# dps/rust-raytracer

Measured on NVIDIA H100. Metric: Mrays/sec (primary+scattered), higher is better.
Workload: dtype f64

## Files before the change

rust-raytracer_b200/csrc/rtb200_api.cu:

```cuda
#include <algorithm>
#include <chrono>
#include <cmath>
#include <cstdio>
#include <cstdlib>
#include <cstring>
#include <mutex>
#include <string>
#include <thread>
#include <vector>

#include "rtb200_bvh.hpp"
#include "rtb200_kernels.cuh"

using namespace rtk;

static_assert(kCapIn >= 32 + 7 * rtbvh::kMaxDepth + 8, "the node stack must hold 32 roots plus a single-entry descent of the deepest tree (LIFO reserve, DESIGN.md 4.1)");

namespace {

thread_local std::string g_last_error;

int fail(int code, const std::string& msg) { g_last_error = msg; return code; }
int fail_cuda(cudaError_t e, const char* what) {
    g_last_error = std::string(what) + ": " + cudaGetErrorName(e) + " (" + cudaGetErrorString(e) + ")";
// ... 406 lines not shown
        const rt_image& im = s->textures[t];
        texs[t].rgb8 = nullptr; texs[t].width = im.width; texs[t].height = im.height;
        if (im.rgb8 && im.width && im.height && im.width * im.height * 3ull <= im.bytes)
            upload_array(h, im.rgb8, im.width * im.height * 3, (void**)&texs[t].rgb8);
    }
    upload_array(h, texs.data(), texs.size() * sizeof(rtd::DevTex), (void**)&tp.tex);
    tp.sky_mode = s->sky.mode;
    tp.sky.rgb8 = nullptr; tp.sky.width = 0; tp.sky.height = 0;
    if (s->sky.mode == RT_SKY_TEXTURE) {
        upload_array(h, s->sky.tex.rgb8, s->sky.tex.width * s->sky.tex.height * 3, (void**)&tp.sky.rgb8);
        tp.sky.width = s->sky.tex.width; tp.sky.height = s->sky.tex.height;
    }
    if (h->mode == MODE_TREE) { h->level_nodes = R.level_nodes; h->level_off = R.level_off; }
    std::vector<uint32_t> lights;
    for (uint32_t i = 0; i < n; ++i) {
        if (s->spheres[i].kind == RT_LIGHT) lights.push_back(i);
        if (albedo_nonfinite(s->spheres[i])) tp.albedo_nonfinite = 1u;
    }
    h->light_idx = lights;
    for (uint64_t t = 0; t < s->n_textures; ++t) h->tex_ok.push_back(image_ok(s->textures[t]));
    lights.push_back(0);
    upload_array(h, lights.data(), lights.size() * 4, (void**)&tp.lights);
    upload_array(h, nullptr, 16, (void**)&h->err);
    upload_array(h, nullptr, kMaxPending * kStatBytes, (void**)&h->stat_snap);
    tp.err = nullptr;
    tp.gx = R.g[0]; tp.gy = R.g[1]; tp.gz = R.g[2];
    tp.er_coef = 1.0f - (float)(96.0 * rtbvh::kU);
    tp.cam = s->camera;
    tp.width = s->width; tp.height = s->height; tp.spp = s->samples_per_pixel; tp.max_depth = s->max_depth;
    tp.key0 = (uint32_t)s->seed; tp.key1 = (uint32_t)(s->seed >> 32);
    tp.rank = opts.rank; tp.world = opts.world; tp.band_rows = opts.band_rows;
    tp.rows_local = rtb200_shard_rows(s->height, opts.rank, opts.world, opts.band_rows);
    tp.npix_local = tp.rows_local * s->width;

    const char* es = getenv("RTB200_WF_SMEM");
    tp.scene_in_smem = es ? (uint32_t)atoi(es) : 0u;
    h->smem = wavefront_smem_bytes(tp, h->mode, tp.scene_in_smem, Q_SINGLE);
    const int occ = occupancy(ctx, h->mode, n_lights > 0, Q_SINGLE, h->smem);
    if (occ <= 0) return fail(RT_ERR_UNSUPPORTED, "no launch configuration fits shared memory");
    h->ctas_per_sm = occ;
    h->grid = ctx->sm_count * occ;

    uint64_t cap = sample_buffer_cap(opts);
    uint64_t per_spp = (uint64_t)std::max<uint32_t>(tp.npix_local, 1) * 16ull;
    uint64_t spb = std::max<uint64_t>(1, cap / per_spp);
    spb = std::min<uint64_t>(spb, s->samples_per_pixel);
    while (spb > 1 && spb * tp.npix_local >= (1ull << 31)) spb /= 2;
    h->spp_batch = (uint32_t)spb;

    if ((rc = commit_uploads(h)) != RT_OK) return rc;
    h->tp.err = h->err;
    guard.ok = true;
    *out = h;
    return RT_OK;
}

int rtb200_scene_upload(const rt_scene* s, const rt_options* opts_in, rtb200_scene_handle* out) {
  return guarded([&]() -> int {
    if (!s || !out) return fail(RT_ERR_INVALID, "null argument");
    *out = nullptr;
    rt_options opts;
    int rc = normalise_options(opts_in, &opts);
    if (rc != RT_OK) return rc;
    uint32_t n_lights = 0;
    if ((rc = validate_scene(s, &n_lights)) != RT_OK) return rc;
    DeviceRestore restore;
// ... 976 lines not shown
```

rust-raytracer_b200/csrc/rtb200_kernels.cuh:

```cuda
#pragma once
#include <cuda_runtime.h>
#include <stdint.h>

#include "../../include/rtb200.h"
#include "rtb200_bvh.hpp"
#include "rtb200_device.cuh"

namespace rtk {

using rtbvh::kLeafK;
constexpr int kNodeVec = rtbvh::kNodeFloats / 4;
constexpr int kChildVec = rtbvh::kChildOff / 4;
using DevMat = rtbvh::Mat32;

#ifndef RT_BLOCK
#define RT_BLOCK 256
#endif
constexpr int kBlock = RT_BLOCK;
#ifndef RT_PHASE_CLOCKS
#define RT_PHASE_CLOCKS 0
#endif
enum : uint32_t { PH_HIT, PH_SORT_WAIT_A, PH_SHADE, PH_REGEN, PH_WAIT_C, PH_ITERS, PH_SCATTERS, PH_DEFERRED,
                  PH_NODE, PH_LEAF, PH_EXACT, PH_EXACT_STEPS, PH_EXACT_TESTS, PH_SRC_SKIPS, kPhaseN };
constexpr uint32_t kPhaseStat = 13;
#ifndef RT_CAP_IN
#define RT_CAP_IN 192
#endif
#ifndef RT_CAP_LF
#define RT_CAP_LF 160
#endif
#ifndef RT_CAP_CD
#define RT_CAP_CD 96
#endif
constexpr int kCapIn = RT_CAP_IN;
constexpr int kCapLf = RT_CAP_LF;
constexpr int kCapCd = RT_CAP_CD;

struct ShadowFrame {
    double px, py, pz;
    double ndx, ndy, ndz;
    float ar, ag, ab;
    float sr, sg, sb;
    uint32_t li, code, is_light, pad;
};
static_assert(sizeof(ShadowFrame) == 88, "ShadowFrame layout");

enum TraceMode : uint32_t { MODE_TREE = 0, MODE_BRUTE = 1, MODE_EXACT = 2 };
enum TraceQueue : uint32_t { Q_SINGLE = 0, Q_FRAMES = 1, Q_LIST = 2 };

struct FrameRec { rt_camera cam; uint32_t key0, key1; };
static_assert(sizeof(FrameRec) == 104, "FrameRec layout");

struct TraceParams {
    const float4*   nodes;
    const float4*   leaf_rec;
    const uint32_t* leaf_id;
    const uint32_t* skip_pos;
    const uint32_t* always;
    const float4*   filt;
    const double4*  geo;
    const DevMat*   mat;
    const rtd::DevTex* tex;
    uint32_t n, n_pairs, n_nodes, n_leaves, n_always, depth;
    uint32_t n_lights;
    uint32_t scene_in_smem;
    double gx, gy, gz;
    float  er_coef;
    rt_camera cam;
    uint32_t width, height, spp, max_depth;
    uint32_t sky_mode;
    rtd::DevTex sky;
    uint32_t key0, key1;
    uint32_t s0, s_count;
    uint32_t npix_local, rows_local;
    int32_t  rank, world;
    uint32_t band_rows;
    uint32_t total_work;
    unsigned int* work_counter;
    float4*  samplebuf;
    uint32_t* stack;
    uint32_t stack_stride;
    const uint32_t* lights;
    ShadowFrame* frames;
    uint32_t max_shadow;
    float* lterm;
    unsigned long long* stat;
    unsigned long long* err;
    const FrameRec* ftab;
    uint32_t frame_work;
    uint32_t albedo_nonfinite;
    const uint32_t* list;
    const uint32_t* list_n;
};

struct AdaptiveParams {
    const float4* samplebuf;
    const uint32_t* list;
    const uint32_t* list_n;
    float* sum;
    float* sq;
    uint32_t* count;
    uint32_t* keep;
    unsigned long long* black_samples;
    uint32_t npix_local, s_count;
    uint32_t n_after;
    uint32_t max_samples, min_samples;
    float abs_tol, rel_tol;
};
struct AdaptiveResolveParams {
    const float* sum; const uint32_t* count;
    uint32_t npix_local;
    float* out_linear; uint8_t* out_rgb8; uint32_t* out_count;
};

struct ResolveParams {
    const float4* samplebuf;
    float*   accum;
    uint32_t npix_local, s_count;
    uint32_t first, last;
    uint32_t spp;
    float*   out_linear;
    uint8_t* out_rgb8;
};

struct RefitParams {
// ... 64 lines not shown
```

rust-raytracer_b200/csrc/rtb200_trace.cuh:

```cuda
#pragma once
#include "rtb200_kernels.cuh"

namespace rtk {

using namespace rtd;

#ifndef RT_SCATTER_TRIPS
#define RT_SCATTER_TRIPS 2
#endif
#ifndef RT_SMEM_STACK
#define RT_SMEM_STACK 10
#endif

enum : uint32_t { CLS_MISS = 0, CLS_DIFFUSE = 1, CLS_METAL = 2, CLS_GLASS = 3, CLS_LIGHT = 4, CLS_DEAD = 5, N_CLS = 6 };
constexpr uint32_t kDeadLevel = 0xffffffffu;
constexpr uint32_t kScatterPending = 0x80000000u;
using rtbvh::kLeafBit;
constexpr unsigned long long kNoHitBits = 0x7ff0000000000000ull;
constexpr uint32_t kNoSphere = 0xffffffffu;
using rtbvh::kSkipNodeBit;
using rtbvh::kNoSkip;
constexpr uint32_t kSlotBytes = 7 * 8 + 10 * 4 + RT_SMEM_STACK * 4;
constexpr uint32_t kFrameSlotBytes = 4;

struct Pool {
    double *ox, *oy, *oz, *dx, *dy, *dz, *bt;
    uint32_t *bi, *work, *pix, *smp, *blk, *clo, *chi, *lvl, *shd;
    uint32_t *src;
    uint32_t *stk;
    uint32_t *frm;
    uint32_t n_slots;
    uint32_t stack_col;
};
RT_DEV Pool pool_at(unsigned char* base, uint32_t n_slots, uint32_t stack_col) {
    Pool P;
    double* d = reinterpret_cast<double*>(base);
    P.ox = d; P.oy = d + n_slots; P.oz = d + 2 * n_slots; P.dx = d + 3 * n_slots; P.dy = d + 4 * n_slots; P.dz = d + 5 * n_slots; P.bt = d + 6 * n_slots;
    uint32_t* u = reinterpret_cast<uint32_t*>(d + 7 * n_slots);
    P.bi = u; P.work = u + n_slots; P.pix = u + 2 * n_slots; P.smp = u + 3 * n_slots; P.blk = u + 4 * n_slots; P.clo = u + 5 * n_slots;
    P.chi = u + 6 * n_slots; P.lvl = u + 7 * n_slots; P.shd = u + 8 * n_slots; P.src = u + 9 * n_slots; P.stk = u + 10 * n_slots;
    P.frm = u + (10 + RT_SMEM_STACK) * n_slots;
    P.n_slots = n_slots; P.stack_col = stack_col;
    return P;
}

struct WarpCtx {
    float4 *cA, *cB, *cC;
    uint32_t *skip;
    uint32_t *l_in, *l_lf, *l_cd;
};
constexpr uint32_t kWarpCtxBytes = 3 * 32 * 16 + 32 * 4 + (uint32_t)(kCapIn + kCapLf + kCapCd) * 4;
RT_DEV WarpCtx warpctx_at(unsigned char* base) {
    WarpCtx W;
    W.cA = reinterpret_cast<float4*>(base); W.cB = W.cA + 32; W.cC = W.cB + 32;
    W.skip = reinterpret_cast<uint32_t*>(W.cC + 32);
    W.l_in = W.skip + 32; W.l_lf = W.l_in + kCapIn; W.l_cd = W.l_lf + kCapLf;
    return W;
}

struct SceneRefs {
    const float4* nodes; const float4* leaf_rec; const uint32_t* leaf_id; const float4* filt;
    const double4* geo; const DevMat* mat;
};

struct Stats {
    uint32_t rays = 0, cand = 0, ovf = 0, samples = 0, leaves = 0, nodes = 0;
#if RT_PHASE_CLOCKS
    unsigned long long t_node = 0, t_leaf = 0, t_exact = 0;
    uint32_t exact_steps = 0, exact_tests = 0, src_skips = 0;
#endif
};

RT_DEV void bulk_stage(void* dst, const void* src, uint32_t bytes, uint64_t* bar) {
    const uint32_t CH = 32768u;
    for (uint32_t o = 0; o < bytes; o += CH) {
        uint32_t nb = bytes - o < CH ? bytes - o : CH;
        tma_bulk_g2s((char*)dst + o, (const char*)src + o, nb, bar);
    }
}

RT_DEV void albedo_of(uint32_t code, const DevMat* mat, float& r, float& g, float& b) {
    if (code == 0xffffffffu) { r = g = b = 1.0f; return; }
    if (code & 0x80000000u) {
        r = __fdiv_rn((float)(code & 0xffu), 255.0f);
        g = __fdiv_rn((float)((code >> 8) & 0xffu), 255.0f);
        b = __fdiv_rn((float)((code >> 16) & 0xffu), 255.0f);
    } else {
        const DevMat& m = mat[code];
        r = m.r; g = m.g; b = m.b;
    }
}

RT_DEV float fmax3(float a, float b, float c) { return fmaxf(fmaxf(a, b), c); }
RT_DEV float fmin3(float a, float b, float c) { return fminf(fminf(a, b), c); }

RT_DEV uint32_t warp_scan_incl(uint32_t v, int lane) {
#pragma unroll
    for (int off = 1; off < 32; off <<= 1) {
        uint32_t t = __shfl_up_sync(0xffffffffu, v, off);
// ... 9 lines not shown
        float4 A_ = (REC)[2 * q], B_ = (REC)[2 * q + 1];                                                                             \
        float2 cx = make_float2(A_.x, A_.y), cy = make_float2(A_.z, A_.w), cz = make_float2(B_.x, B_.y), nk = make_float2(B_.z, B_.w); \
        float2 bb = fma2_rn(cz, dz2, nod2);                                                                                          \
        float2 tt = fma2_rn(cz, oz2, nk);                                                                                            \
        bb = fma2_rn(cy, dy2, bb);                                                                                                   \
        tt = fma2_rn(cy, oy2, tt);                                                                                                   \
        bb = fma2_rn(cx, dx2, bb);                                                                                                   \
        tt = fma2_rn(cx, ox2, tt);                                                                                                   \
        (DV)[q] = fma2_rn(bb, bb, tt);                                                                                               \
    }

RT_DEV uint32_t class_of(uint32_t kind) {
    return (kind == RT_METAL) ? CLS_METAL : (kind == RT_GLASS) ? CLS_GLASS : (kind == RT_LIGHT) ? CLS_LIGHT : CLS_DIFFUSE;
}

template <uint32_t MODE>
RT_DEV uint32_t closest_hit(const TraceParams& p, const SceneRefs& sc, const Pool& P, const WarpCtx& W, bool alive, uint32_t slot, int lane, Stats& st) {
    const unsigned FULL = 0xffffffffu;
    uint32_t cls = CLS_DEAD;
    if (__ballot_sync(FULL, alive) == 0u) return cls;
    const uint32_t lt_mask = (1u << lane) - 1u;
    unsigned long long* btu = reinterpret_cast<unsigned long long*>(P.bt);
    const D3 o = mk(P.ox[slot], P.oy[slot], P.oz[slot]), d = mk(P.dx[slot], P.dy[slot], P.dz[slot]);
    const double a = length_squared(d);
    bool ovf = false;
    double best_t = DBL_MAX;
    int best = -1;
    auto confirm = [&](int j) {
        double4 gq = sc.geo[j];
        double root;
        if (sphere_root(mk(gq.x, gq.y, gq.z), gq.w, o, d, a, 0.001, DBL_MAX, root)) {
            if (best < 0 || root < best_t || (root == best_t && j < best)) { best_t = root; best = j; }
        }
        ++st.cand;
    };
    if (alive) { btu[slot] = kNoHitBits; P.bi[slot] = 0xffffffffu; }
    if (MODE != MODE_EXACT) {
        const float ofx = __double2float_rn(__dsub_rn(o.x, p.gx)), ofy = __double2float_rn(__dsub_rn(o.y, p.gy)),
                    ofz = __double2float_rn(__dsub_rn(o.z, p.gz));
        const float dfx = __double2float_rn(d.x), dfy = __double2float_rn(d.y), dfz = __double2float_rn(d.z);
        const float s = fmaf(dfx, dfx, fmaf(dfy, dfy, dfz * dfz));
        const float oo = fmaf(ofx, ofx, fmaf(ofy, ofy, ofz * ofz));
        const bool ok = (s > 1e-30f) && (s < 1e30f) && (oo < 1e30f);
        const float inv = rsqrtf(s);
        const float dnx = dfx * inv, dny = dfy * inv, dnz = dfz * inv;
        const float nod = -fmaf(ofx, dnx, fmaf(ofy, dny, ofz * dnz));
        const float thr = __fmul_rd(oo, p.er_coef);
        if (alive && !ok) ovf = true;
        if (MODE == MODE_TREE) {
            const float ax = fabsf(dnx) < 1e-20f ? copysignf(1e-20f, dnx) : dnx;
            const float ay = fabsf(dny) < 1e-20f ? copysignf(1e-20f, dny) : dny;
            const float az = fabsf(dnz) < 1e-20f ? copysignf(1e-20f, dnz) : dnz;
            const float mray = __fmul_ru(1.9073486328125e-6f, __fsqrt_ru(oo));
            W.cA[lane] = make_float4(ofx, ofy, ofz, mray);
            W.cB[lane] = make_float4(__frcp_rn(ax), __frcp_rn(ay), __frcp_rn(az), thr);
            W.cC[lane] = make_float4(dnx, dny, dnz, nod);
            uint32_t skp = kNoSkip;
            const uint32_t src = alive ? P.src[slot] : kNoSphere;
            if (src != kNoSphere) {
                const uint32_t pos = p.skip_pos[src];
                const double4 gs = sc.geo[src];
                if (pos != kNoSkip && leaves_sphere(mk(gs.x, gs.y, gs.z), gs.w, o, d, a)) skp = pos;
            }
            W.skip[lane] = skp;
            const uint32_t fat_in = (uint32_t)kCapIn - 7u * p.depth - 8u;
            const bool enter = alive && ok && p.n_nodes != 0u;
            const unsigned em = __ballot_sync(FULL, enter);
// ... 44 lines not shown
                                   ((R1.x >> 31) << 4) | ((R1.y >> 31) << 5) | ((R1.z >> 31) << 6) | ((R1.w >> 31) << 7);
                    }
                    {
                        const uint32_t sk = W.skip[ray] ^ (kSkipNodeBit | node << 3);
                        if (sk < 8u) {
#if RT_PHASE_CLOCKS
                            st.src_skips += (hit >> sk) & 1u;
#endif
                            hit &= ~(1u << sk);
                        }
                    }
                    const uint32_t packed = (uint32_t)__popc(hit & ~leafbits) | ((uint32_t)__popc(hit & leafbits) << 16);
                    const uint32_t inc = warp_scan_incl(packed, lane);
                    const uint32_t new_in = n_in - ((uint32_t)lane + 1u) + (inc & 0xffffu);
                    const bool fits = new_in <= (lane == 0 ? (uint32_t)kCapIn : fat_in) && n_lf + (inc >> 16) <= (uint32_t)kCapLf;
                    const unsigned okm = __ballot_sync(FULL, fits || !act);
                    uint32_t k = okm == FULL ? 32u : (uint32_t)(__ffs(~okm) - 1);
                    k = k < m ? k : m;
                    if (k == 0u) { if (lane == 0) atomicAdd(&p.err[1], 1ull); break; }
                    const uint32_t tot = __shfl_sync(FULL, inc, (int)k - 1);
                    __syncwarp();
                    if (act && (uint32_t)lane < k) {
                        const uint32_t exc = inc - packed;
                        uint32_t pi = (n_in - k) + (exc & 0xffffu), pl = n_lf + (exc >> 16);
                        const uint32_t* refs = reinterpret_cast<const uint32_t*>(N + kChildVec);
                        uint32_t mm = hit;
                        while (mm) {
                            const int c = __ffs(mm) - 1;
                            mm &= mm - 1u;
                            const uint32_t ref = refs[c];
                            if (ref & kLeafBit) W.l_lf[pl++] = (ref << 5) | ray;
                            else W.l_in[pi++] = (ref << 5) | ray;
                        }
                        ++st.nodes;
                    }
                    n_in = n_in - k + (tot & 0xffffu);
                    n_lf += tot >> 16;
                    __syncwarp();
#if RT_PHASE_CLOCKS
                    if (lane == 0) st.t_node += clock64() - t_step;
#endif
                } else if (n_lf != 0u && n_cd <= (uint32_t)(kCapCd - 32)) {
                    const uint32_t m = n_lf < 32u ? n_lf : 32u;
                    const bool act = (uint32_t)lane < m;
                    const uint32_t e = act ? W.l_lf[n_lf - 1u - (uint32_t)lane] : 0u;
                    const uint32_t ray = e & 31u, leaf = e >> 5;
                    uint32_t hit = 0u;
                    if (act) {
                        const float4 A = W.cA[ray], C = W.cC[ray];
                        const float th = W.cB[ray].w;
                        const float2 dx2 = make_float2(C.x, C.x), dy2 = make_float2(C.y, C.y), dz2 = make_float2(C.z, C.z);
                        const float2 ox2 = make_float2(2.f * A.x, 2.f * A.x), oy2 = make_float2(2.f * A.y, 2.f * A.y), oz2 = make_float2(2.f * A.z, 2.f * A.z);
                        const float2 nod2 = make_float2(C.w, C.w);
                        float2 Dv[kLeafK / 2];
                        const float4* rec = sc.leaf_rec + (size_t)leaf * kLeafK;
                        RT_FILTER_PAIRS(rec, Dv, kLeafK / 2)
#pragma unroll
                        for (int q = 0; q < kLeafK / 2; ++q) hit |= (Dv[q].x >= th ? 1u : 0u) << (2 * q) | (Dv[q].y >= th ? 1u : 0u) << (2 * q + 1);
                        const uint32_t sk = W.skip[ray];
                        if (sk / (uint32_t)kLeafK == leaf) {
#if RT_PHASE_CLOCKS
                            st.src_skips += (hit >> (sk % (uint32_t)kLeafK)) & 1u;
#endif
                            hit &= ~(1u << (sk % (uint32_t)kLeafK));
                        }
                    }
                    const uint32_t cntc = (uint32_t)__popc(hit);
                    const uint32_t inc = warp_scan_incl(cntc, lane);
                    const bool fits = n_cd + inc <= (uint32_t)kCapCd;
                    const unsigned okm = __ballot_sync(FULL, fits || !act);
                    uint32_t k = okm == FULL ? 32u : (uint32_t)(__ffs(~okm) - 1);
                    k = k < m ? k : m;
                    if (k == 0u) { if (lane == 0) atomicAdd(&p.err[1], 1ull); break; }
                    const uint32_t tot = __shfl_sync(FULL, inc, (int)k - 1);
                    if (act && (uint32_t)lane < k) {
                        uint32_t pc = n_cd + inc - cntc;
                        const uint32_t* ids = sc.leaf_id + (size_t)leaf * kLeafK;
                        uint32_t mm = hit;
                        while (mm) {
                            const int c = __ffs(mm) - 1;
                            mm &= mm - 1u;
                            W.l_cd[pc++] = (ids[c] << 5) | ray;
                        }
                        ++st.leaves;
                    }
                    n_lf -= k;
                    n_cd += tot;
                    __syncwarp();
#if RT_PHASE_CLOCKS
                    if (lane == 0) st.t_leaf += clock64() - t_step;
#endif
                } else if (n_cd != 0u) {
                    const uint32_t m = n_cd < 32u ? n_cd : 32u;
                    const bool act = (uint32_t)lane < m;
                    const uint32_t e = act ? W.l_cd[n_cd - 1u - (uint32_t)lane] : 0u;
                    const uint32_t rs = __shfl_sync(FULL, slot, (int)(e & 31u)), sph = e >> 5;
                    unsigned long long key = ~0ull;
                    if (act) {
                        const D3 ro = mk(P.ox[rs], P.oy[rs], P.oz[rs]), rd = mk(P.dx[rs], P.dy[rs], P.dz[rs]);
                        const double4 gq = sc.geo[sph];
                        double root;
                        if (sphere_root(mk(gq.x, gq.y, gq.z), gq.w, ro, rd, length_squared(rd), 0.001, DBL_MAX, root)) key = (unsigned long long)__double_as_longlong(root);
                        ++st.cand;
#if RT_PHASE_CLOCKS
                        ++st.exact_tests;
#endif
                    }
                    const bool h = key != ~0ull;
                    const unsigned long long before = h ? btu[rs] : 0ull;
                    __syncwarp();
                    if (h && key < before) atomicMin(&btu[rs], key);
                    __syncwarp();
                    const bool mine = h && key == btu[rs];
                    if (mine && key < before) atomicMax(&P.bi[rs], 0xffffffffu);
                    __syncwarp();
                    if (mine) atomicMin(&P.bi[rs], sph);
                    n_cd -= m;
                    __syncwarp();
#if RT_PHASE_CLOCKS
                    if (lane == 0) { st.t_exact += clock64() - t_step; ++st.exact_steps; }
#endif
                } else {
                    break;
                }
                if (++guard > (1u << 22)) { if (lane == 0) atomicAdd(&p.err[1], 1ull); break; }
            }
        } else {
            if (alive && ok) {
                const float2 dx2 = make_float2(dnx, dnx), dy2 = make_float2(dny, dny), dz2 = make_float2(dnz, dnz);
                const float2 ox2 = make_float2(2.f * ofx, 2.f * ofx), oy2 = make_float2(2.f * ofy, 2.f * ofy), oz2 = make_float2(2.f * ofz, 2.f * ofz);
                const float2 nod2 = make_float2(nod, nod);
#pragma unroll 1
                for (uint32_t pp = 0; pp < p.n_pairs; pp += 4) {
                    float2 Dv[4];
                    const float4* rec = sc.filt + 2 * pp;
                    RT_FILTER_PAIRS(rec, Dv, 4)
#pragma unroll
                    for (int q = 0; q < 4; ++q) {
                        const uint32_t j = 2u * (pp + (uint32_t)q);
                        if (Dv[q].x >= thr && j < p.n) confirm((int)j);
                        if (Dv[q].y >= thr && j + 1u < p.n) confirm((int)j + 1);
                    }
                }
            }
        }
    } else {
        ovf = alive;
    }
    if (alive) {
        if (ovf) {
            ++st.ovf;
            for (int k = 0; k < (int)p.n; ++k) confirm(k);
        } else if (MODE == MODE_TREE) {
            for (uint32_t k = 0; k < p.n_always; ++k) confirm((int)p.always[k]);
        }
        const unsigned long long tb = btu[slot];
        const uint32_t ti = P.bi[slot];
        if (best >= 0) {
            const unsigned long long kb = (unsigned long long)__double_as_longlong(best_t);
            if (ti == 0xffffffffu || kb < tb || (kb == tb && (uint32_t)best < ti)) { P.bt[slot] = best_t; P.bi[slot] = (uint32_t)best; }
        }
        const uint32_t fin = P.bi[slot];
        cls = CLS_MISS;
        if (fin != 0xffffffffu) cls = class_of(sc.mat[fin].kind);
        ++st.rays;
    }
    return cls;
}

template <bool LIGHTS, uint32_t QUEUE>
RT_DEV bool regenerate_slot(const TraceParams& p, const Pool& P, bool want, uint32_t s, int lane, bool& exhausted, Stats& st,
                            uint32_t n_list = 0u) {
    constexpr bool FRAMES = QUEUE == Q_FRAMES;
    const unsigned FULL = 0xffffffffu;
    want = want && !exhausted;
    unsigned need = __ballot_sync(FULL, want);
    if (!need) return false;
    int leader = __ffs(need) - 1;
    unsigned base = 0;
    if (lane == leader) base = atomicAdd(p.work_counter, (unsigned)__popc(need));
    base = __shfl_sync(FULL, base, leader);
    if (base + (unsigned)__popc(need) >= (QUEUE == Q_LIST ? n_list * p.s_count : p.total_work)) exhausted = true;
    if (!want) return false;
    unsigned my = base + __popc(need & ((1u << lane) - 1u));
    if (my >= (QUEUE == Q_LIST ? n_list * p.s_count : p.total_work)) return false;
    uint32_t f = 0u, k0 = p.key0, k1 = p.key1;
    if constexpr (FRAMES) { f = my / p.frame_work; my -= f * p.frame_work; k0 = p.ftab[f].key0; k1 = p.ftab[f].key1; }
    uint32_t x, s_local, y_local, lp, k_list = 0u;
    if constexpr (QUEUE == Q_LIST) {
        s_local = my % p.s_count;
        k_list = n_list - 1u - my / p.s_count;
        lp = p.list[k_list];
        y_local = lp / p.width;
        x = lp - y_local * p.width;
    } else {
        x = my % p.width;
        const uint32_t t_ = my / p.width;
        s_local = t_ % p.s_count;
        const uint32_t rr = t_ / p.s_count;
        y_local = p.rows_local - 1u - rr;
        lp = y_local * p.width + x;
    }
    uint32_t band = y_local / p.band_rows;
    uint32_t y = (band * (uint32_t)p.world + (uint32_t)p.rank) * p.band_rows + (y_local - band * p.band_rows);
    Rng rng; rng_init(rng, y * p.width + x, p.s0 + s_local);
    double xi1 = rng_f64(rng, k0, k1);
    double u = __ddiv_rn(__dadd_rn((double)x, xi1), __dsub_rn((double)p.width, 1.0));
    double xi2 = rng_f64(rng, k0, k1);
    double v = __ddiv_rn(__dsub_rn((double)p.height, __dadd_rn((double)y, xi2)), __dsub_rn((double)p.height, 1.0));
    D3 o, d;
    if constexpr (FRAMES) get_ray(p.ftab[f].cam, u, v, o, d);
    else get_ray(p.cam, u, v, o, d);
    P.ox[s] = o.x; P.oy[s] = o.y; P.oz[s] = o.z; P.dx[s] = d.x; P.dy[s] = d.y; P.dz[s] = d.z;
    if constexpr (FRAMES) { P.work[s] = (f * p.s_count + s_local) * p.npix_local + lp; P.frm[s] = f; }
    else if constexpr (QUEUE == Q_LIST) P.work[s] = s_local * n_list + k_list;
    else P.work[s] = s_local * p.npix_local + lp;
    P.pix[s] = rng.pixel; P.smp[s] = rng.sample;
    P.blk[s] = (rng.blk << 1) | rng.has; P.clo[s] = rng.c_lo; P.chi[s] = rng.c_hi;
    P.lvl[s] = 0u;
    P.shd[s] = 0u;
    P.src[s] = kNoSphere;
    if (LIGHTS) {
        for (int q = 0; q < 6; ++q) p.lterm[(size_t)q * p.stack_stride + P.stack_col + s] = 0.0f;
    }
    ++st.samples;
    return true;
}

template <bool LIGHTS, bool FRAMES>
RT_DEV bool shade_slot(const TraceParams& p, const SceneRefs& sc, const Pool& P, uint32_t s, uint32_t c) {
    uint32_t k0 = p.key0, k1 = p.key1;
    if constexpr (FRAMES) { const FrameRec& fr = p.ftab[P.frm[s]]; k0 = fr.key0; k1 = fr.key1; }
    const DevMat* mat = sc.mat;
    const double4* geo = sc.geo;
    const size_t col = (size_t)P.stack_col + s;
    auto stack_push = [&](uint32_t lvl, uint32_t code) {
        if (lvl < (uint32_t)RT_SMEM_STACK) P.stk[lvl * P.n_slots + s] = code; else p.stack[(size_t)lvl * p.stack_stride + col] = code;
    };
    auto stack_get = [&](uint32_t lvl) -> uint32_t {
        return lvl < (uint32_t)RT_SMEM_STACK ? P.stk[lvl * P.n_slots + s] : p.stack[(size_t)lvl * p.stack_stride + col];
    };
    Rng rng; rng.pixel = P.pix[s]; rng.sample = P.smp[s];
    { uint32_t bh = P.blk[s]; rng.blk = bh >> 1; rng.has = bh & 1u; }
    rng.c_lo = P.clo[s]; rng.c_hi = P.chi[s];
    bool done = false;
    D3 o = mk(P.ox[s], P.oy[s], P.oz[s]), d = mk(P.dx[s], P.dy[s], P.dz[s]);
    uint32_t level = P.lvl[s];
    uint32_t shd = LIGHTS ? (P.shd[s] & ~kScatterPending) : 0u;
    const uint32_t rays_sample = level + 1u;
    float cr = 0.f, cg = 0.f, cb = 0.f;
    bool have_tc = false;
    float tr = 0.f, tg = 0.f, tb = 0.f;
    bool state_dirty = false;
    if (c == CLS_MISS) {
        float x, y, z;
        sky_color(d, length(d), p.sky_mode, p.sky, x, y, z);
        if (shd == 0u) { cr = x; cg = y; cb = z; done = true; }
        else { tr = x; tg = y; tb = z; have_tc = true; }
    } else {
        const uint32_t best = P.bi[s];
        const double best_t = P.bt[s];
        double4 gq = geo[best];
        const D3 center = mk(gq.x, gq.y, gq.z);
        HitRec h = hit_record(center, gq.w, o, d, best_t);
        const DevMat m = mat[best];
        uint32_t code = best;
        D3 nd = d;
        bool absorbed = false;
        const bool is_light = (c == CLS_LIGHT);
        D3 rs = mk(0, 0, 0);
        if (c == CLS_DIFFUSE || c == CLS_METAL) {
            const unsigned group = __activemask();
            const bool sampled = random_in_unit_sphere_ilp<RT_SCATTER_TRIPS>(rng, k0, k1, rs);
            __syncwarp(group);
            if (!sampled) {
// ... 103 lines not shown
                    tr = clampf(__fadd_rn(Lr, __fmul_rn(f.ar, 0.0f))); tg = clampf(__fadd_rn(Lg, __fmul_rn(f.ag, 0.0f))); tb = clampf(__fadd_rn(Lb, __fmul_rn(f.ab, 0.0f)));
                }
            }
        }
    }
    if (state_dirty && !done) {
        P.ox[s] = o.x; P.oy[s] = o.y; P.oz[s] = o.z; P.dx[s] = d.x; P.dy[s] = d.y; P.dz[s] = d.z;
        P.blk[s] = (rng.blk << 1) | rng.has; P.clo[s] = rng.c_lo; P.chi[s] = rng.c_hi;
        P.lvl[s] = level;
        P.shd[s] = shd;
    }
    if (done) {
        if (LIGHTS || p.albedo_nonfinite || cr != 0.f || cg != 0.f || cb != 0.f) {
            for (int l = (int)level - 1; l >= 0; --l) {
                float ar, ag, ab;
                albedo_of(stack_get((uint32_t)l), mat, ar, ag, ab);
                float Lr = 0.f, Lg = 0.f, Lb = 0.f;
                if (LIGHTS && l < 2) {
                    Lr = p.lterm[(size_t)(l * 3 + 0) * p.stack_stride + col];
                    Lg = p.lterm[(size_t)(l * 3 + 1) * p.stack_stride + col];
                    Lb = p.lterm[(size_t)(l * 3 + 2) * p.stack_stride + col];
                }
                cr = clampf(__fadd_rn(Lr, __fmul_rn(ar, cr)));
                cg = clampf(__fadd_rn(Lg, __fmul_rn(ag, cg)));
                cb = clampf(__fadd_rn(Lb, __fmul_rn(ab, cb)));
            }
        }
        p.samplebuf[P.work[s]] = make_float4(cr, cg, cb, __uint_as_float(rays_sample));
        P.lvl[s] = kDeadLevel;
    }
    return done;
}

RT_DEV void flush_stats(const TraceParams& p, const Stats& st, int lane) {
    unsigned long long v[6] = {st.rays, st.cand, st.ovf, st.samples, st.leaves, st.nodes};
#pragma unroll
    for (int k = 0; k < 6; ++k) {
#pragma unroll
        for (int off = 16; off > 0; off >>= 1) v[k] += __shfl_down_sync(0xffffffffu, v[k], off);
    }
    if (lane == 0) {
        atomicAdd(&p.stat[0], v[0]);
        atomicAdd(&p.stat[1], v[1]);
        atomicAdd(&p.stat[2], v[2]);
        atomicAdd(&p.stat[3], v[3]);
        atomicAdd(&p.stat[4], v[4]);
        atomicAdd(&p.stat[6], v[5]);
    }
#if RT_PHASE_CLOCKS
    unsigned long long w[6] = {st.t_node, st.t_leaf, st.t_exact, st.exact_steps, st.exact_tests, st.src_skips};
#pragma unroll
    for (int k = 0; k < 6; ++k) {
#pragma unroll
        for (int off = 16; off > 0; off >>= 1) w[k] += __shfl_down_sync(0xffffffffu, w[k], off);
    }
    if (lane == 0) {
#pragma unroll
        for (int k = 0; k < 6; ++k) atomicAdd(&p.stat[kPhaseStat + PH_NODE + k], w[k]);
    }
#endif
}

}
```

rust-raytracer_b200/csrc/rtb200_wavefront.cu:

```cuda
#include <cstdio>
#include <cstdlib>

#include "rtb200_trace.cuh"

namespace rtk {

namespace {

struct WfSmem {
    uint32_t nodes_off, leafrec_off, leafid_off, filt_off, geo_off, mat_off;
    uint32_t warpctx;
    uint32_t pool;
    uint32_t perm;
    uint32_t cnt;
    uint32_t phase;
    uint32_t total;
};

__host__ __device__ constexpr WfSmem wf_layout(uint32_t n, uint32_t n_pairs, uint32_t n_nodes, uint32_t n_leaves, uint32_t mode, uint32_t mask, bool frames) {
    WfSmem L{};
    uint32_t off = 16;
    L.nodes_off = off;   if (mode == MODE_TREE && (mask & 1u)) off += n_nodes * (uint32_t)(kNodeVec * 16);
    L.leafrec_off = off; if (mode == MODE_TREE && (mask & 1u)) off += n_leaves * (uint32_t)(kLeafK * 16);
    L.leafid_off = off;  if (mode == MODE_TREE && (mask & 1u)) off += n_leaves * (uint32_t)(kLeafK * 4);
// ... 60 lines not shown
    sc.mat = (p.scene_in_smem & 4u) ? reinterpret_cast<const DevMat*>(smem_raw + L.mat_off) : p.mat;
    const int tid = threadIdx.x;
    const int lane = tid & 31;
    const unsigned FULL = 0xffffffffu;
    const Pool P = pool_at(smem_raw + L.pool, (uint32_t)kBlock, blockIdx.x * (uint32_t)kBlock);
    const WarpCtx W = warpctx_at(smem_raw + L.warpctx + (uint32_t)(tid >> 5) * kWarpCtxBytes);
    uint16_t* s_perm = reinterpret_cast<uint16_t*>(smem_raw + L.perm);
    uint32_t* s_cnt = reinterpret_cast<uint32_t*>(smem_raw + L.cnt);

    if (tid == 0) mbar_init(bar, 1);
    if (tid < 16) s_cnt[tid] = 0;
    P.lvl[tid] = kDeadLevel;
    __syncthreads();
    if (tid == 0) {
        const uint32_t b_nodes = (MODE == MODE_TREE && tree_smem) ? p.n_nodes * (uint32_t)(kNodeVec * 16) : 0u;
        const uint32_t b_lrec = (MODE == MODE_TREE && tree_smem) ? p.n_leaves * (uint32_t)(kLeafK * 16) : 0u;
        const uint32_t b_lid = (MODE == MODE_TREE && tree_smem) ? p.n_leaves * (uint32_t)(kLeafK * 4) : 0u;
        const uint32_t b_filt = (MODE == MODE_BRUTE && tree_smem) ? p.n_pairs * 32u : 0u;
        const uint32_t b_geo = (p.scene_in_smem & 2u) ? p.n * 32u : 0u, b_mat = (p.scene_in_smem & 4u) ? p.n * 32u : 0u;
        mbar_arrive_expect_tx(bar, b_nodes + b_lrec + b_lid + b_filt + b_geo + b_mat);
        if (b_nodes) bulk_stage(smem_raw + L.nodes_off, p.nodes, b_nodes, bar);
        if (b_lrec) bulk_stage(smem_raw + L.leafrec_off, p.leaf_rec, b_lrec, bar);
        if (b_lid) bulk_stage(smem_raw + L.leafid_off, p.leaf_id, b_lid, bar);
        if (b_filt) bulk_stage(smem_raw + L.filt_off, p.filt, b_filt, bar);
        if (b_geo) bulk_stage(smem_raw + L.geo_off, p.geo, b_geo, bar);
        if (b_mat) bulk_stage(smem_raw + L.mat_off, p.mat, b_mat, bar);
    }
    mbar_wait(bar, 0);

    auto now_ns = []() { unsigned long long t; asm volatile("mov.u64 %0, %%globaltimer;" : "=l"(t)); return t; };
    if (tid == 0) atomicMin(&p.stat[8], now_ns());
    Stats st;
    bool exhausted = false;
    bool stamped = false;
    uint32_t dry_iters = 0;
    uint32_t n_list = 0u;
    if constexpr (QUEUE == Q_LIST) n_list = *p.list_n;
    regenerate_slot<LIGHTS, QUEUE>(p, P, true, (uint32_t)tid, lane, exhausted, st, n_list);
    __syncthreads();

#if RT_PHASE_CLOCKS
    static_assert(kPhaseStat + kPhaseN <= 32, "the per-launch stat block holds 32 counters");
    unsigned long long* ph = reinterpret_cast<unsigned long long*>(smem_raw + L.phase) + (uint32_t)(tid >> 5) * kPhaseN;
    if (lane < (int)kPhaseN) ph[lane] = 0ull;
    unsigned long long t_mark = clock64();
    auto tick = [&](uint32_t k) { __syncwarp(); const unsigned long long t = clock64(); if (lane == 0) ph[k] += t - t_mark; t_mark = t; };
#endif
    const uint32_t lt_mask = (1u << lane) - 1u;
    uint32_t it = 0;
    for (;; ++it) {
        uint32_t* cnt = s_cnt + (it & 1u) * 8u;
        const bool alive = P.lvl[tid] != kDeadLevel;
        const bool pending = alive && (P.shd[tid] & kScatterPending) != 0u;
        uint32_t cls = closest_hit<MODE>(p, sc, P, W, alive && !pending, (uint32_t)tid, lane, st);
        if (pending) cls = class_of(sc.mat[P.bi[tid]].kind);
#if RT_PHASE_CLOCKS
        tick(PH_HIT);
#endif

#pragma unroll
        for (uint32_t c = 0; c < CLS_DEAD; ++c) {
            unsigned b = __ballot_sync(FULL, cls == c);
            if (b) {
                uint32_t base = 0;
                if (lane == 0) base = atomicAdd(&cnt[c], (uint32_t)__popc(b));
                base = __shfl_sync(FULL, base, 0);
                if (cls == c) s_perm[c * (uint32_t)kBlock + base + (uint32_t)__popc(b & lt_mask)] = (uint16_t)tid;
            }
        }
        __syncthreads();
#if RT_PHASE_CLOCKS
        tick(PH_SORT_WAIT_A);
#endif
        uint32_t c0 = cnt[0], c1 = cnt[1], c2 = cnt[2], c3 = cnt[3], c4 = cnt[4];
        const uint32_t e0 = c0, e1 = e0 + c1, e2 = e1 + c2, e3 = e2 + c3, n_live = e3 + c4;
        if (tid < 8) s_cnt[((it + 1u) & 1u) * 8u + tid] = 0u;

        const bool active = (uint32_t)tid < n_live;
        const uint32_t c = !active ? CLS_DEAD : ((uint32_t)tid < e0 ? CLS_MISS : (uint32_t)tid < e1 ? CLS_DIFFUSE : (uint32_t)tid < e2 ? CLS_METAL : (uint32_t)tid < e3 ? CLS_GLASS : CLS_LIGHT);
        const uint32_t cstart = c == CLS_MISS ? 0u : c == CLS_DIFFUSE ? e0 : c == CLS_METAL ? e1 : c == CLS_GLASS ? e2 : e3;
        const uint32_t s = active ? (uint32_t)s_perm[c * (uint32_t)kBlock + ((uint32_t)tid - cstart)] : 0u;
        bool done = false;
        if (active) done = shade_slot<LIGHTS, FRAMES>(p, sc, P, s, c);
#if RT_PHASE_CLOCKS
        tick(PH_SHADE);
        {
            const bool scatter = active && (c == CLS_DIFFUSE || c == CLS_METAL);
            const unsigned sm = __ballot_sync(FULL, scatter), dm = __ballot_sync(FULL, scatter && !done && (P.shd[s] & kScatterPending) != 0u);
            if (lane == 0) { ph[PH_ITERS] += 1ull; ph[PH_SCATTERS] += (unsigned)__popc(sm); ph[PH_DEFERRED] += (unsigned)__popc(dm); }
        }
#endif
        regenerate_slot<LIGHTS, QUEUE>(p, P, active && done, s, lane, exhausted, st, n_list);
        if (exhausted && !stamped) { stamped = true; if (lane == 0) atomicMin(&p.stat[9], now_ns()); }
        if (stamped) ++dry_iters;
        const bool still_alive = active && (P.lvl[s] != kDeadLevel);
#if RT_PHASE_CLOCKS
        tick(PH_REGEN);
#endif
        const int more = __syncthreads_or(still_alive ? 1 : 0);
#if RT_PHASE_CLOCKS
        tick(PH_WAIT_C);
#endif
        if (!more) break;
    }
    flush_stats(p, st, lane);
#if RT_PHASE_CLOCKS
    __syncwarp();
    if (lane < (int)kPhaseN) atomicAdd(&p.stat[kPhaseStat + lane], ph[lane]);
#endif
    if (tid == 0) { atomicMax(&p.stat[10], now_ns()); atomicMax(&p.stat[11], (unsigned long long)dry_iters); atomicAdd(&p.stat[12], (unsigned long long)dry_iters); }
}

template <uint32_t QUEUE, typename F>
static auto dispatch_mode(uint32_t mode, bool lights, F&& f) {
    if (mode == MODE_EXACT) return lights ? f(rt_wavefront_kernel<MODE_EXACT, true, QUEUE>) : f(rt_wavefront_kernel<MODE_EXACT, false, QUEUE>);
    if (mode == MODE_BRUTE) return lights ? f(rt_wavefront_kernel<MODE_BRUTE, true, QUEUE>) : f(rt_wavefront_kernel<MODE_BRUTE, false, QUEUE>);
    return lights ? f(rt_wavefront_kernel<MODE_TREE, true, QUEUE>) : f(rt_wavefront_kernel<MODE_TREE, false, QUEUE>);
}
template <typename F>
static auto dispatch(uint32_t mode, bool lights, uint32_t queue, F&& f) {
    if (queue == Q_LIST) return dispatch_mode<Q_LIST>(mode, lights, f);
    return queue == Q_FRAMES ? dispatch_mode<Q_FRAMES>(mode, lights, f) : dispatch_mode<Q_SINGLE>(mode, lights, f);
}

cudaError_t launch_wavefront(const TraceParams& p, uint32_t mode, uint32_t queue, int grid, size_t smem, cudaStream_t st) {
    return dispatch(mode, p.n_lights > 0, queue, [&](auto kern) -> cudaError_t {
        cudaError_t e = cudaFuncSetAttribute(kern, cudaFuncAttributeMaxDynamicSharedMemorySize, (int)smem);
        if (e == cudaSuccess) e = set_carveout(kern, mode, smem);
        if (e != cudaSuccess) return e;
        kern<<<grid, kBlock, smem, st>>>(p);
        return cudaGetLastError();
    });
}

int wavefront_max_ctas_per_sm(uint32_t mode, bool lights, uint32_t queue, size_t smem) {
    return dispatch(mode, lights, queue, [&](auto kern) -> int {
        int nb = 0;
        if (cudaFuncSetAttribute(kern, cudaFuncAttributeMaxDynamicSharedMemorySize, (int)smem) != cudaSuccess) { cudaGetLastError(); return 0; }
        if (set_carveout(kern, mode, smem) != cudaSuccess) { cudaGetLastError(); return 0; }
        if (cudaOccupancyMaxActiveBlocksPerMultiprocessor(&nb, kern, kBlock, smem) != cudaSuccess) { cudaGetLastError(); return 0; }
        return nb;
    });
// ... 17 lines not shown
```

Baseline: 5655.

## Recompute pixel/sample from work index and compress per-thread stats counters

Removes the per-slot pixel and sample arrays from the shared-memory pool and recomputes them from the work index at shade time using precomputed magic-number division. The freed slot bytes go to a larger shared-memory traversal stack. Per-thread statistics counters are collapsed into one lane-indexed accumulator, and some candidate counts are derived analytically at flush time, to reduce register pressure and per-ray increments. The cost is extra integer arithmetic in shading, and the stats semantics change slightly.

```diff
diff --git a/rust-raytracer_b200/csrc/rtb200_api.cu b/rust-raytracer_b200/csrc/rtb200_api.cu
--- a/rust-raytracer_b200/csrc/rtb200_api.cu
+++ b/rust-raytracer_b200/csrc/rtb200_api.cu
@@ -462,6 +462,7 @@
     tp.rank = opts.rank; tp.world = opts.world; tp.band_rows = opts.band_rows;
     tp.rows_local = rtb200_shard_rows(s->height, opts.rank, opts.world, opts.band_rows);
     tp.npix_local = tp.rows_local * s->width;
+    tp.npix_magic = fastdiv_magic(tp.npix_local); tp.width_magic = fastdiv_magic(tp.width); tp.band_magic = fastdiv_magic(tp.band_rows);
 
     const char* es = getenv("RTB200_WF_SMEM");
     tp.scene_in_smem = es ? (uint32_t)atoi(es) : 0u;
diff --git a/rust-raytracer_b200/csrc/rtb200_kernels.cuh b/rust-raytracer_b200/csrc/rtb200_kernels.cuh
--- a/rust-raytracer_b200/csrc/rtb200_kernels.cuh
+++ b/rust-raytracer_b200/csrc/rtb200_kernels.cuh
@@ -51,6 +51,11 @@
 struct FrameRec { rt_camera cam; uint32_t key0, key1; };
 static_assert(sizeof(FrameRec) == 104, "FrameRec layout");
 
+__host__ __device__ inline unsigned long long fastdiv_magic(uint32_t d) { return d > 1u ? ~0ull / d + 1ull : 0ull; }
+__device__ __forceinline__ uint32_t fastdiv_u32(uint32_t n, uint32_t d, unsigned long long magic) {
+    return d > 1u ? (uint32_t)__umul64hi((unsigned long long)n, magic) : n;
+}
+
 struct TraceParams {
     const float4*   nodes;
     const float4*   leaf_rec;
@@ -91,6 +96,7 @@
     uint32_t albedo_nonfinite;
     const uint32_t* list;
     const uint32_t* list_n;
+    unsigned long long npix_magic, width_magic, band_magic;
 };
 
 struct AdaptiveParams {
diff --git a/rust-raytracer_b200/csrc/rtb200_trace.cuh b/rust-raytracer_b200/csrc/rtb200_trace.cuh
--- a/rust-raytracer_b200/csrc/rtb200_trace.cuh
+++ b/rust-raytracer_b200/csrc/rtb200_trace.cuh
@@ -9,7 +9,7 @@
 #define RT_SCATTER_TRIPS 2
 #endif
 #ifndef RT_SMEM_STACK
-#define RT_SMEM_STACK 10
+#define RT_SMEM_STACK 12
 #endif
 
 enum : uint32_t { CLS_MISS = 0, CLS_DIFFUSE = 1, CLS_METAL = 2, CLS_GLASS = 3, CLS_LIGHT = 4, CLS_DEAD = 5, N_CLS = 6 };
@@ -20,12 +20,12 @@
 constexpr uint32_t kNoSphere = 0xffffffffu;
 using rtbvh::kSkipNodeBit;
 using rtbvh::kNoSkip;
-constexpr uint32_t kSlotBytes = 7 * 8 + 10 * 4 + RT_SMEM_STACK * 4;
+constexpr uint32_t kSlotBytes = 7 * 8 + 8 * 4 + RT_SMEM_STACK * 4;
 constexpr uint32_t kFrameSlotBytes = 4;
 
 struct Pool {
     double *ox, *oy, *oz, *dx, *dy, *dz, *bt;
-    uint32_t *bi, *work, *pix, *smp, *blk, *clo, *chi, *lvl, *shd;
+    uint32_t *bi, *work, *blk, *clo, *chi, *lvl, *shd;
     uint32_t *src;
     uint32_t *stk;
     uint32_t *frm;
@@ -37,9 +37,9 @@
     double* d = reinterpret_cast<double*>(base);
     P.ox = d; P.oy = d + n_slots; P.oz = d + 2 * n_slots; P.dx = d + 3 * n_slots; P.dy = d + 4 * n_slots; P.dz = d + 5 * n_slots; P.bt = d + 6 * n_slots;
     uint32_t* u = reinterpret_cast<uint32_t*>(d + 7 * n_slots);
-    P.bi = u; P.work = u + n_slots; P.pix = u + 2 * n_slots; P.smp = u + 3 * n_slots; P.blk = u + 4 * n_slots; P.clo = u + 5 * n_slots;
-    P.chi = u + 6 * n_slots; P.lvl = u + 7 * n_slots; P.shd = u + 8 * n_slots; P.src = u + 9 * n_slots; P.stk = u + 10 * n_slots;
-    P.frm = u + (10 + RT_SMEM_STACK) * n_slots;
+    P.bi = u; P.work = u + n_slots; P.blk = u + 2 * n_slots; P.clo = u + 3 * n_slots;
+    P.chi = u + 4 * n_slots; P.lvl = u + 5 * n_slots; P.shd = u + 6 * n_slots; P.src = u + 7 * n_slots; P.stk = u + 8 * n_slots;
+    P.frm = u + (8 + RT_SMEM_STACK) * n_slots;
     P.n_slots = n_slots; P.stack_col = stack_col;
     return P;
 }
@@ -63,8 +63,11 @@
     const double4* geo; const DevMat* mat;
 };
 
+enum : uint32_t { SC_RAYS = 0, SC_CAND = 1, SC_OVF = 2, SC_SAMPLES = 3, SC_LEAVES = 4, SC_NODES = 5, SC_N = 6 };
 struct Stats {
-    uint32_t rays = 0, cand = 0, ovf = 0, samples = 0, leaves = 0, nodes = 0;
+    uint32_t acc = 0;
+    uint32_t cand_lane = 0;
+    RT_DEV void add(int lane, uint32_t k, uint32_t v) { acc += (uint32_t)lane == k ? v : 0u; }
 #if RT_PHASE_CLOCKS
     unsigned long long t_node = 0, t_leaf = 0, t_exact = 0;
     uint32_t exact_steps = 0, exact_tests = 0, src_skips = 0;
@@ -140,7 +143,7 @@
         if (sphere_root(mk(gq.x, gq.y, gq.z), gq.w, o, d, a, 0.001, DBL_MAX, root)) {
             if (best < 0 || root < best_t || (root == best_t && j < best)) { best_t = root; best = j; }
         }
-        ++st.cand;
+        if (MODE == MODE_BRUTE) ++st.cand_lane;
     };
     if (alive) { btu[slot] = kNoHitBits; P.bi[slot] = 0xffffffffu; }
     if (MODE != MODE_EXACT) {
@@ -251,8 +254,8 @@
                             if (ref & kLeafBit) W.l_lf[pl++] = (ref << 5) | ray;
                             else W.l_in[pi++] = (ref << 5) | ray;
                         }
-                        ++st.nodes;
-                    }
+                    }
+                    st.add(lane, SC_NODES, k);
                     n_in = n_in - k + (tot & 0xffffu);
                     n_lf += tot >> 16;
                     __syncwarp();
@@ -301,8 +304,8 @@
                             mm &= mm - 1u;
                             W.l_cd[pc++] = (ids[c] << 5) | ray;
                         }
-                        ++st.leaves;
-                    }
+                    }
+                    st.add(lane, SC_LEAVES, k);
                     n_lf -= k;
                     n_cd += tot;
                     __syncwarp();
@@ -320,7 +323,6 @@
                         const double4 gq = sc.geo[sph];
                         double root;
                         if (sphere_root(mk(gq.x, gq.y, gq.z), gq.w, ro, rd, length_squared(rd), 0.001, DBL_MAX, root)) key = (unsigned long long)__double_as_longlong(root);
-                        ++st.cand;
 #if RT_PHASE_CLOCKS
                         ++st.exact_tests;
 #endif
@@ -334,6 +336,7 @@
                     if (mine && key < before) atomicMax(&P.bi[rs], 0xffffffffu);
                     __syncwarp();
                     if (mine) atomicMin(&P.bi[rs], sph);
+                    st.add(lane, SC_CAND, m);
                     n_cd -= m;
                     __syncwarp();
 #if RT_PHASE_CLOCKS
@@ -368,7 +371,6 @@
     }
     if (alive) {
         if (ovf) {
-            ++st.ovf;
             for (int k = 0; k < (int)p.n; ++k) confirm(k);
         } else if (MODE == MODE_TREE) {
             for (uint32_t k = 0; k < p.n_always; ++k) confirm((int)p.always[k]);
@@ -382,8 +384,9 @@
         const uint32_t fin = P.bi[slot];
         cls = CLS_MISS;
         if (fin != 0xffffffffu) cls = class_of(sc.mat[fin].kind);
-        ++st.rays;
-    }
+    }
+    st.add(lane, SC_RAYS, (uint32_t)__popc(__ballot_sync(FULL, alive)));
+    st.add(lane, SC_OVF, (uint32_t)__popc(__ballot_sync(FULL, ovf)));
     return cls;
 }
 
@@ -399,10 +402,12 @@
     unsigned base = 0;
     if (lane == leader) base = atomicAdd(p.work_counter, (unsigned)__popc(need));
     base = __shfl_sync(FULL, base, leader);
-    if (base + (unsigned)__popc(need) >= (QUEUE == Q_LIST ? n_list * p.s_count : p.total_work)) exhausted = true;
+    const unsigned limit = QUEUE == Q_LIST ? n_list * p.s_count : p.total_work;
+    if (base + (unsigned)__popc(need) >= limit) exhausted = true;
+    st.add(lane, SC_SAMPLES, base >= limit ? 0u : min((unsigned)__popc(need), limit - base));
     if (!want) return false;
     unsigned my = base + __popc(need & ((1u << lane) - 1u));
-    if (my >= (QUEUE == Q_LIST ? n_list * p.s_count : p.total_work)) return false;
+    if (my >= limit) return false;
     uint32_t f = 0u, k0 = p.key0, k1 = p.key1;
     if constexpr (FRAMES) { f = my / p.frame_work; my -= f * p.frame_work; k0 = p.ftab[f].key0; k1 = p.ftab[f].key1; }
     uint32_t x, s_local, y_local, lp, k_list = 0u;
@@ -434,7 +439,6 @@
     if constexpr (FRAMES) { P.work[s] = (f * p.s_count + s_local) * p.npix_local + lp; P.frm[s] = f; }
     else if constexpr (QUEUE == Q_LIST) P.work[s] = s_local * n_list + k_list;
     else P.work[s] = s_local * p.npix_local + lp;
-    P.pix[s] = rng.pixel; P.smp[s] = rng.sample;
     P.blk[s] = (rng.blk << 1) | rng.has; P.clo[s] = rng.c_lo; P.chi[s] = rng.c_hi;
     P.lvl[s] = 0u;
     P.shd[s] = 0u;
@@ -442,14 +446,35 @@
     if (LIGHTS) {
         for (int q = 0; q < 6; ++q) p.lterm[(size_t)q * p.stack_stride + P.stack_col + s] = 0.0f;
     }
-    ++st.samples;
     return true;
 }
 
-template <bool LIGHTS, bool FRAMES>
-RT_DEV bool shade_slot(const TraceParams& p, const SceneRefs& sc, const Pool& P, uint32_t s, uint32_t c) {
-    uint32_t k0 = p.key0, k1 = p.key1;
-    if constexpr (FRAMES) { const FrameRec& fr = p.ftab[P.frm[s]]; k0 = fr.key0; k1 = fr.key1; }
+template <uint32_t QUEUE>
+RT_DEV void rng_coords(const TraceParams& p, uint32_t work, uint32_t f, uint32_t n_list, unsigned long long list_magic,
+                       uint32_t& pixel, uint32_t& sample) {
+    uint32_t s_local, lp;
+    if constexpr (QUEUE == Q_LIST) {
+        s_local = fastdiv_u32(work, n_list, list_magic);
+        lp = p.list[work - s_local * n_list];
+    } else {
+        const uint32_t t = fastdiv_u32(work, p.npix_local, p.npix_magic);
+        lp = work - t * p.npix_local;
+        s_local = QUEUE == Q_FRAMES ? t - f * p.s_count : t;
+    }
+    const uint32_t y_local = fastdiv_u32(lp, p.width, p.width_magic);
+    const uint32_t x = lp - y_local * p.width;
+    const uint32_t band = fastdiv_u32(y_local, p.band_rows, p.band_magic);
+    const uint32_t y = (band * (uint32_t)p.world + (uint32_t)p.rank) * p.band_rows + (y_local - band * p.band_rows);
+    pixel = y * p.width + x;
+    sample = p.s0 + s_local;
+}
+
+template <bool LIGHTS, uint32_t QUEUE>
+RT_DEV bool shade_slot(const TraceParams& p, const SceneRefs& sc, const Pool& P, uint32_t s, uint32_t c, uint32_t n_list = 0u,
+                       unsigned long long list_magic = 0ull) {
+    constexpr bool FRAMES = QUEUE == Q_FRAMES;
+    uint32_t k0 = p.key0, k1 = p.key1, f = 0u;
+    if constexpr (FRAMES) { f = P.frm[s]; const FrameRec& fr = p.ftab[f]; k0 = fr.key0; k1 = fr.key1; }
     const DevMat* mat = sc.mat;
     const double4* geo = sc.geo;
     const size_t col = (size_t)P.stack_col + s;
@@ -459,7 +484,8 @@
     auto stack_get = [&](uint32_t lvl) -> uint32_t {
         return lvl < (uint32_t)RT_SMEM_STACK ? P.stk[lvl * P.n_slots + s] : p.stack[(size_t)lvl * p.stack_stride + col];
     };
-    Rng rng; rng.pixel = P.pix[s]; rng.sample = P.smp[s];
+    Rng rng;
+    rng_coords<QUEUE>(p, P.work[s], f, n_list, list_magic, rng.pixel, rng.sample);
     { uint32_t bh = P.blk[s]; rng.blk = bh >> 1; rng.has = bh & 1u; }
     rng.c_lo = P.clo[s]; rng.c_hi = P.chi[s];
     bool done = false;
@@ -629,29 +655,26 @@
     return done;
 }
 
+template <uint32_t MODE>
 RT_DEV void flush_stats(const TraceParams& p, const Stats& st, int lane) {
-    unsigned long long v[6] = {st.rays, st.cand, st.ovf, st.samples, st.leaves, st.nodes};
+    unsigned long long cand = st.cand_lane;
+#pragma unroll
+    for (int off = 16; off > 0; off >>= 1) cand += __shfl_xor_sync(0xffffffffu, cand, off);
+    const uint32_t rays = __shfl_sync(0xffffffffu, st.acc, SC_RAYS), ovf = __shfl_sync(0xffffffffu, st.acc, SC_OVF);
+    if (MODE != MODE_BRUTE) cand = (unsigned long long)ovf * p.n;
+    if (MODE == MODE_TREE) cand += (unsigned long long)(rays - ovf) * p.n_always;
+    if ((uint32_t)lane < SC_N) {
+        const unsigned long long v = st.acc + (lane == (int)SC_CAND ? cand : 0ull);
+        atomicAdd(&p.stat[lane == (int)SC_NODES ? 6 : lane], v);
+    }
+#if RT_PHASE_CLOCKS
+    unsigned long long w[6] = {st.t_node, st.t_leaf, st.t_exact, st.exact_steps, st.exact_tests, st.src_skips};
 #pragma unroll
     for (int k = 0; k < 6; ++k) {
 #pragma unroll
-        for (int off = 16; off > 0; off >>= 1) v[k] += __shfl_down_sync(0xffffffffu, v[k], off);
+        for (int off = 16; off > 0; off >>= 1) w[k] += __shfl_down_sync(0xffffffffu, w[k], off);
     }
     if (lane == 0) {
-        atomicAdd(&p.stat[0], v[0]);
-        atomicAdd(&p.stat[1], v[1]);
-        atomicAdd(&p.stat[2], v[2]);
-        atomicAdd(&p.stat[3], v[3]);
-        atomicAdd(&p.stat[4], v[4]);
-        atomicAdd(&p.stat[6], v[5]);
-    }
-#if RT_PHASE_CLOCKS
-    unsigned long long w[6] = {st.t_node, st.t_leaf, st.t_exact, st.exact_steps, st.exact_tests, st.src_skips};
-#pragma unroll
-    for (int k = 0; k < 6; ++k) {
-#pragma unroll
-        for (int off = 16; off > 0; off >>= 1) w[k] += __shfl_down_sync(0xffffffffu, w[k], off);
-    }
-    if (lane == 0) {
 #pragma unroll
         for (int k = 0; k < 6; ++k) atomicAdd(&p.stat[kPhaseStat + PH_NODE + k], w[k]);
     }
diff --git a/rust-raytracer_b200/csrc/rtb200_wavefront.cu b/rust-raytracer_b200/csrc/rtb200_wavefront.cu
--- a/rust-raytracer_b200/csrc/rtb200_wavefront.cu
+++ b/rust-raytracer_b200/csrc/rtb200_wavefront.cu
@@ -116,10 +116,10 @@
     if (tid == 0) atomicMin(&p.stat[8], now_ns());
     Stats st;
     bool exhausted = false;
-    bool stamped = false;
-    uint32_t dry_iters = 0;
+    uint32_t it_dry = ~0u;
     uint32_t n_list = 0u;
-    if constexpr (QUEUE == Q_LIST) n_list = *p.list_n;
+    unsigned long long list_magic = 0ull;
+    if constexpr (QUEUE == Q_LIST) { n_list = *p.list_n; list_magic = fastdiv_magic(n_list); }
     regenerate_slot<LIGHTS, QUEUE>(p, P, true, (uint32_t)tid, lane, exhausted, st, n_list);
     __syncthreads();
 
@@ -165,7 +165,7 @@
         const uint32_t cstart = c == CLS_MISS ? 0u : c == CLS_DIFFUSE ? e0 : c == CLS_METAL ? e1 : c == CLS_GLASS ? e2 : e3;
         const uint32_t s = active ? (uint32_t)s_perm[c * (uint32_t)kBlock + ((uint32_t)tid - cstart)] : 0u;
         bool done = false;
-        if (active) done = shade_slot<LIGHTS, FRAMES>(p, sc, P, s, c);
+        if (active) done = shade_slot<LIGHTS, QUEUE>(p, sc, P, s, c, n_list, list_magic);
 #if RT_PHASE_CLOCKS
         tick(PH_SHADE);
         {
@@ -175,8 +175,7 @@
         }
 #endif
         regenerate_slot<LIGHTS, QUEUE>(p, P, active && done, s, lane, exhausted, st, n_list);
-        if (exhausted && !stamped) { stamped = true; if (lane == 0) atomicMin(&p.stat[9], now_ns()); }
-        if (stamped) ++dry_iters;
+        if (exhausted && it_dry == ~0u) { it_dry = it; if (lane == 0) atomicMin(&p.stat[9], now_ns()); }
         const bool still_alive = active && (P.lvl[s] != kDeadLevel);
 #if RT_PHASE_CLOCKS
         tick(PH_REGEN);
@@ -187,11 +186,12 @@
 #endif
         if (!more) break;
     }
-    flush_stats(p, st, lane);
+    flush_stats<MODE>(p, st, lane);
 #if RT_PHASE_CLOCKS
     __syncwarp();
     if (lane < (int)kPhaseN) atomicAdd(&p.stat[kPhaseStat + lane], ph[lane]);
 #endif
+    const uint32_t dry_iters = it_dry == ~0u ? 0u : it - it_dry + 1u;
     if (tid == 0) { atomicMax(&p.stat[10], now_ns()); atomicMax(&p.stat[11], (unsigned long long)dry_iters); atomicAdd(&p.stat[12], (unsigned long long)dry_iters); }
 }
 
```

After: 5672 (median of 6 runs). About the same (+0.3%).
